# CrazeXD/Prometheus

Hardware: AMD Instinct MI355X
Metric: spectrum points/sec (phase x wavelength) (higher is better)
Workload: dtype f64; 1 GPU; C3 (powerLaw: NaI+CaII+MgI), 351222 wavelengths x 16 phases x 2400 chords x 30 samples; global_wavelengths=351222, orbital_phases=16, chords_per_phase=2400, los_samples=30, parallelism=wavelength shards x1 (no collective)

## Files before the change

### prometheus_amd/csrc/prom_api.hip

```cpp
#include <algorithm>
#include <cstdio>
#include <cstdlib>
#include <cmath>
#include <cstring>
#include <exception>
#include <map>
#include <mutex>
#include <thread>

#include "prom_internal.h"

using prom::DevBuf;
using prom::Error;

namespace {

template <class F>
int32_t guarded(prom_ctx* ctx, F&& f) {
  if (!ctx) return PROM_E_ARG;
  try {
    PROM_HIP(hipSetDevice(ctx->device));
    f();
    ctx->err.clear();
    return PROM_OK;
// ... 699 lines not shown
          double m = 0.0;
          const int64_t cnt = n_orb * tr.n_pr * tr.n_x;
          for (int64_t i = 0; i < cnt; ++i) {
            const double v = std::fabs(S.n_tabulated[i]);
            if (std::isfinite(v) && v > m) m = v;
          }
          nref[sc] = m;
        } else if (S.density.kind == PROM_DENSITY_GRIDDED) {
          int64_t gnx, gny, gnz, glen;
          gridded_dims(S.density, &gnx, &gny, &gnz, &glen);
          double m = 0.0;
          for (int64_t i = gnx + gny + gnz; i < glen; ++i) {
            const double v = std::fabs(S.n_tabulated[i]);
            if (std::isfinite(v) && v > m) m = v;
          }
          nref[sc] = m * (1.0 + 1e-9);
        } else {
          const double* p = S.density.p;
          bool bounded = p[0] >= 0.0 && std::isfinite(p[0]);
          if (S.density.kind == PROM_DENSITY_BAROMETRIC) bounded = bounded && p[2] > 0.0;
          if (S.density.kind == PROM_DENSITY_POWERLAW) bounded = bounded && p[2] >= 0.0 && p[1] > 0.0;
          if (S.density.kind == PROM_DENSITY_HYDROSTATIC)
            bounded = bounded && p[4] >= 0.0 && p[1] > 0.0 && p[3] != 0.0 &&
                      p[4] >= p[2] / (p[3] * p[1]) * (1.0 - 1e-12);
          if (!bounded) tr.window = false;
          nref[sc] = std::fabs(p[0]) * (1.0 + 1e-9);
        }
      }
      for (const auto& t : tr.terms)
        if (!t.is_molecule && !(t.chi >= 0.0)) tr.window = false;
      std::vector<prom::SigTabDev> st;
      for (const auto& t : tr.terms) {
        if (t.is_molecule) continue;
        const prom::AtomTable& tb = ctx->tables[t.table];
        const double bound = std::fabs(t.chi) * nref[t.scenario] * (double)tr.n_x * tr.delta_x;
        const double c = (bound > 0.0 && std::isfinite(bound)) ? 1.0 / bound : 0.0;
        if (!std::isfinite(bound) || (bound > 0.0 && !(c > 0.0))) tr.window = false;
        const double inv = (c > 0.0 && std::isfinite(c)) ? bound : 0.0;
        st.push_back({tb.x.as<double>(), tb.y.as<double>(), tb.n, tb.offset,
                      tr.shift.as<double>() + (int64_t)t.scenario * n_orb, tb.dir.as<int32_t>(), tb.n_dir, 0,
                      tb.dir_x0, tb.dir_inv_h, std::isfinite(c) ? c : 0.0, inv, t.chi, tb.hx.front(), tb.hx.back(),
                      tb.rec.as<double4>()});
      }
      int32_t sc0 = -1;
      bool one_sc = n_atoms >= 2 && n_mol == 0;
      double smax_m = 0.0;
      for (const auto& t : tr.terms) {
        if (t.is_molecule) continue;
        if (sc0 < 0) sc0 = t.scenario;
        if (t.scenario != sc0 || !(std::isfinite(t.chi) && t.chi >= 0.0)) one_sc = false;
        smax_m += t.chi * tr.atom_sigma_max[t.slot];
      }
      tr.species_merge_ok = tr.species_merge_ok && one_sc && tr.n_sc <= 4;
      if (tr.species_merge_ok) {
        const double bound = nref[sc0] * (double)tr.n_x * tr.delta_x;
        const double c = (bound > 0.0 && std::isfinite(bound)) ? 1.0 / bound : 0.0;
        if (!std::isfinite(bound) || (bound > 0.0 && !(c > 0.0)) || !std::isfinite(smax_m)) tr.species_merge_ok = false;
        tr.sigtab_m = prom::SigTabs4{};
        tr.sigtab_m.t[0] = st[0];
        tr.sigtab_m.t[0].ncoef = std::isfinite(c) ? c : 0.0;
        tr.sigtab_m.t[0].nscale = (c > 0.0 && std::isfinite(c)) ? bound : 0.0;
        tr.sigtab_m.t[0].chi = 1.0;
        tr.colargs_m = prom::ColArgs{};
        prom::TermDev tm{};
        tm.scenario = sc0;
        tm.is_molecule = 0;
        tm.slot = 0;
        tm.table = -1;
        tm.chi = 1.0;
        tr.colargs_m.t[0] = tm;
        stg.add(tr.sigma_max_m, &smax_m, 1, s);
        tr.qbound_m = smax_m * tr.sigtab_m.t[0].nscale;
      }
      stg.add(tr.sigtab, st.data(), (int64_t)st.size(), s);
      tr.qbound_v = 0.0;
      for (size_t i = 0; i < st.size(); ++i) tr.qbound_v += tr.atom_sigma_max[i] * st[i].nscale;
      {
        const bool cols8e = n_mol == 0 && tr.n_x <= 64 && (int32_t)tr.terms.size() <= 8 && tr.n_sc <= 4;
        tr.tcurve = tr.tcurve && cols8e && tr.exp_mode && tr.window && !pb->has_star && n_atoms >= 1 &&
                    (n_atoms == 1 || tr.species_merge_ok);
        const double yb = !tr.tcurve ? 0.0 : (n_atoms == 1 ? tr.atom_sigma_max[0] : smax_m);
        const double nb = !tr.tcurve ? 0.0 : (n_atoms == 1 ? st[0].nscale : tr.sigtab_m.t[0].nscale);
        tr.tc_ybound = (std::isfinite(yb) && yb > 0.0) ? yb : 0.0;
        const double qb = yb * nb;
        int lg = prom::kTcMaxOctaves;
        if (std::isfinite(qb) && qb > 0.0) lg = std::max(1, std::min(prom::kTcMaxOctaves, std::ilogb(qb) + 7 + 2));
        if (const char* e = std::getenv("PROM_TC_LG")) lg = std::max(1, std::min(lg, std::atoi(e)));
        tr.tc_lg = lg;
      }
      tr.uniform_shift = !(pb->options & PROM_OPT_DOPPLER_ROWS);
      for (const auto& t : tr.terms) {
        if (t.is_molecule) continue;
        for (int64_t o = 1; o < n_orb; ++o)
          if (!(sh[t.scenario * n_orb + o] == sh[t.scenario * n_orb])) tr.uniform_shift = false;
      }
      tr.sigtab_v = prom::SigTabs4{};
      for (size_t i = 0; i < st.size() && i < 4; ++i) tr.sigtab_v.t[i] = st[i];
      tr.sig_seg_ok = false;
      std::vector<double> key_sh;
      std::vector<uint64_t> key_gen;
      for (const auto& t : tr.terms) {
        if (t.is_molecule) continue;
        key_gen.push_back(ctx->tables[t.table].gen);
        key_sh.insert(key_sh.end(), sh.begin() + t.scenario * n_orb, sh.begin() + (t.scenario + 1) * n_orb);
      }
      const char* srows = std::getenv("PROM_SIGMA_ROWS");
      const bool no_guess = srows && std::atoi(srows) == 0;
      const char* e_sd = std::getenv("PROM_SEG_DIR");
      const bool use_dir = !(e_sd && std::atoi(e_sd) == 0);
      const bool want_seg = true;
      const bool seg_reuse = !no_guess && use_dir && tr.seg_key_valid && key_gen == tr.seg_key_gen &&
                             key_sh == tr.seg_key_sh && (int64_t)tr.seg_key_wav.size() == tr.n_wav &&
                             std::memcmp(tr.seg_key_wav.data(), pb->wavelength, sizeof(double) * tr.n_wav) == 0;
      tr.seg_key_valid = false;
      seg_key_keep = seg_reuse;
      if (!seg_reuse) tr.tw_ok = false;
      const char* e_tw = std::getenv("PROM_TW");
      const bool tw_off = e_tw && std::atoi(e_tw) == 0;
      auto build_tw = [&]() {
        tr.tw_ok = false;
        tr.n_tw = 0;
        std::vector<const std::vector<double>*> tabs;
        int32_t sc_tw = -1;
        bool one = n_orb >= 2;
        for (const auto& t : tr.terms) {
          if (t.is_molecule) continue;
          if (sc_tw < 0) sc_tw = t.scenario;
          for (int64_t o = 0; o < n_orb; ++o)
            if (!(sh[t.scenario * n_orb + o] == sh[sc_tw * n_orb + o])) one = false;
          tabs.push_back(&ctx->tables[t.table].hx);
        }
        if (!one || sc_tw < 0 || tw_off) return;
        static const int rowcap_env = [] { const char* e = std::getenv("PROM_TW_ROWCAP"); return e ? std::max(1, std::atoi(e)) : 0; }();
        const int rowcap = rowcap_env > 0 ? rowcap_env : std::max(256, std::min(768, (int)(4096 / std::max<int64_t>(1, n_orb)) / 64 * 64));
        static const int64_t pmax_env = [] { const char* e = std::getenv("PROM_TW_PMAX"); return e ? (int64_t)std::max(1, std::atoi(e)) : (int64_t)0; }();
        const int64_t pmax = pmax_env > 0 ? pmax_env : std::max<int64_t>(8192, (int64_t)rowcap * n_orb);
        static const int lamcap = [] {
          const char* e = std::getenv("PROM_TW_LAMCAP");
          return e ? std::max(0, std::min(prom::kTwLamCap, std::atoi(e))) : prom::kTwLamCap;
        }();
        static const int lds = [] {
          const char* e = std::getenv("PROM_TW_LDS");
          return e ? std::max(16, std::min(prom::kTwLds, std::atoi(e))) : prom::kTwLds;
        }();
        std::vector<prom::SigSeg> twseg;
        std::vector<int32_t> twrow, twlam;
        int32_t nw = 0;
        if (!prom::build_target_windows(pb->wavelength, tr.n_wav, sh.data() + (int64_t)sc_tw * n_orb, (int32_t)n_orb, tabs,
                                        lds, lamcap, rowcap, pmax, twseg, twrow, twlam, nw))
          return;
        stg.add(tr.tw_seg, twseg.data(), (int64_t)twseg.size(), s);
        stg.add(tr.tw_row, twrow.data(), (int64_t)twrow.size(), s);
        stg.add(tr.tw_lam, twlam.data(), (int64_t)twlam.size(), s);
        tr.n_tw = nw;
        tr.tw_ok = true;
        tr.tw_new = true;
        if (std::getenv("PROM_DEBUG")) {
          int64_t k[4] = {0, 0, 0, 0};
          for (const auto& e : twseg) k[e.kind & 3] += 1;
          int64_t lam_st = 0, lam_n = 0;
          for (int32_t b = 0; b < nw; ++b)
            if (twlam[2 * b + 1] > twlam[2 * b]) {
              ++lam_st;
              lam_n += twlam[2 * b + 1] - twlam[2 * b];
            }
          std::fprintf(stderr, "[prom] target windows: %d (slices: %lld staged, %lld global, %lld staged unguessed, "
                       "%lld outside the table; wavelengths staged in %lld windows, %.1f per window)\n", nw,
                       (long long)k[1], (long long)k[2], (long long)k[3], (long long)k[0], (long long)lam_st,
                       lam_st ? (double)lam_n / (double)lam_st : 0.0);
        }
      };
      if (seg_reuse) {
        tr.sig_seg_ok = true;
        if (tw_off) tr.tw_ok = false;
        else if (!tr.tw_ok) build_tw();
      } else if (want_seg && n_atoms >= 1 && n_atoms <= 4) {
        tr.seg_key_valid = false;
        const int64_t nb = (tr.n_wav + prom::kSigBlockW - 1) / prom::kSigBlockW;
        std::vector<prom::SigSeg> seg(nb * n_atoms, prom::SigSeg{0, 0, 0, 0, 0.0, 0.0});
        std::vector<prom::SigSeg> seg4(nb * n_atoms * 4, prom::SigSeg{0, 0, 0, 0, 0.0, 0.0});
        std::vector<prom::SigSeg> segr;
        std::vector<int32_t> sdir;
        std::mutex segr_mu;
        int32_t ia = 0;
        for (const auto& t : tr.terms) {
          if (t.is_molecule) continue;
          const prom::AtomTable& tb = ctx->tables[t.table];
          const std::vector<double>& X = tb.hx;
          const int64_t n = tb.n;
          double smin = INFINITY, smax = -INFINITY;
          bool ok = n >= 2 && (int64_t)X.size() == n;
          for (int64_t o = 0; o < n_orb; ++o) {
            const double v = sh[t.scenario * n_orb + o];
            if (!(v > 0.0) || !std::isfinite(v)) ok = false;
            smin = std::min(smin, v);
            smax = std::max(smax, v);
          }
          auto bracket = [&](double v) -> int64_t {
            int64_t j = (int64_t)(std::upper_bound(X.begin(), X.end(), v) - X.begin()) - 1;
            return j < 0 ? 0 : (j > n - 2 ? n - 2 : j);
          };
          auto make_seg = [&](double tlo, double thi, prom::SigSeg& e) -> bool {
            const int64_t lo = bracket(tlo);
            const int64_t hi = bracket(thi) + 1;
            const int64_t m = hi - lo + 1;
            if (m < 2 || m > INT32_MAX / 2) return false;
            e.lo = (int32_t)lo;
            e.m = (int32_t)m;
            const double xs = X[lo], span = X[hi] - X[lo];
            const double inv = span > 0.0 ? (double)(m - 1) / span : 0.0;
            const double b0 = -(xs * inv);
            bool lin = span > 0.0 && std::isfinite(inv) && std::isfinite(b0);
            auto guess = [&](double v) -> int64_t {
              const double f = std::fma(v, inv, b0);
              int64_t g = f < 0.0 ? 0 : (f >= (double)(m - 2) ? m - 2 : (int64_t)f);
              return g;
            };
            for (int64_t i = lo; lin && i < hi; ++i) {
              if (X[i] == X[i + 1]) continue;
              const double a = std::max(X[i], tlo), z = std::nextafter(X[i + 1], -INFINITY);
              if (a > z) continue;
              const int64_t k = i - lo;
              const int64_t ga = guess(a), gz = guess(z);
              if (ga < k - 1 || ga > k + 1 || gz < k - 1 || gz > k + 1) lin = false;
            }
            e.kind = 0;
            if (lin) {
              e.kind = (m <= prom::kSigSeg ? 1 : 2) | (m <= prom::tc_slice_cap(n_atoms) ? 64 : 0);
              e.xs = b0;
              e.inv = inv;
            }
            return true;
          };
          auto blocks = [&](int64_t b0, int64_t b1) {
          for (int64_t b = b0; ok && b < b1; ++b) {
            double lmin = INFINITY, lmax = -INFINITY;
            bool fin = true;
            for (int64_t w = b * prom::kSigBlockW; w < std::min<int64_t>(tr.n_wav, (b + 1) * prom::kSigBlockW); ++w) {
              const double l = pb->wavelength[w];
              if (!(l > 0.0) || !std::isfinite(l)) fin = false;
              lmin = std::min(lmin, l);
              lmax = std::max(lmax, l);
            }
            if (!fin) continue;
            const double tlo = smin * lmin, thi = smax * lmax;
            if (!(tlo >= X[0] && thi < X[n - 1])) continue;
            prom::SigSeg& e = seg[b * n_atoms + ia];
            if (!make_seg(tlo, thi, e)) continue;
            if ((e.kind & 3) == 0) {
              bool any = false;
              for (int q = 0; q < prom::kSigBlockW / 64; ++q) {
                double wl = INFINITY, wh = -INFINITY;
                const int64_t w0 = b * prom::kSigBlockW + 64 * q;
                for (int64_t w = w0; w < std::min<int64_t>(tr.n_wav, w0 + 64); ++w) {
                  wl = std::min(wl, pb->wavelength[w]);
                  wh = std::max(wh, pb->wavelength[w]);
                }
                prom::SigSeg& ew = seg4[(b * n_atoms + ia) * 4 + q];
                if (wl <= wh && make_seg(smin * wl, smax * wh, ew) && (ew.kind & 3) != 0) {
                  ew.kind = 2;
                  any = true;
                } else {
                  ew = prom::SigSeg{0, 0, 0, 0, 0.0, 0.0};
                }
              }
              if (any) e.kind |= 8;
              if (!use_dir) continue;
              const int64_t lo = e.lo, m = e.m, hi = lo + m - 1;
              const double x0 = X[lo], span = X[hi] - X[lo];
              if (!(span > 0.0)) continue;
              std::vector<int32_t> dv;
              prom::SigSeg de{(int32_t)lo, 0, 32, 0, 0.0, 0.0};
              bool okd = false;
              for (int64_t mult = 4; !okd && mult <= 1024 && m * mult <= (1 << 22); mult *= 4) {
                const int64_t B = m * mult;
                const double inv = (double)B / span, b0 = -(x0 * inv);
                if (!std::isfinite(inv) || !std::isfinite(b0)) break;
                dv.assign(B, 0);
                int64_t k = 0;
                for (int64_t j = 0; j < B; ++j) {
                  const double v = x0 + span * ((double)j / (double)B);
                  while (k < m - 2 && X[lo + k + 1] <= v) ++k;
                  dv[j] = (int32_t)k;
                }
                auto gd = [&](double v) -> int64_t {
                  const double f = std::fma(v, inv, b0);
                  const int64_t j = f < 0.0 ? 0 : (f >= (double)(B - 1) ? B - 1 : (int64_t)f);
                  return dv[j];
                };
                okd = true;
                for (int64_t o = 0; okd && o < n_orb; ++o) {
                  const double v = sh[t.scenario * n_orb + o];
                  for (int64_t w = b * prom::kSigBlockW; okd && w < (b + 1) * prom::kSigBlockW; ++w) {
                    const double tt = v * pb->wavelength[std::min<int64_t>(w, tr.n_wav - 1)];
                    const int64_t kk = bracket(tt) - lo, g = gd(tt);
                    if (kk < 0 || kk > m - 2 || g < kk - 1 || g > kk + 1) okd = false;
                  }
                }
                if (okd) {
                  de.m = (int32_t)(B + 1);
                  de.xs = b0;
                  de.inv = inv;
                }
              }
              if (okd) {
                std::lock_guard<std::mutex> lk(segr_mu);
// ... 626 lines not shown
```

### prometheus_amd/csrc/prom_internal.h

```cpp
#pragma once

#include <hip/hip_runtime.h>

#include <cstdint>
#include <stdexcept>
#include <string>
#include <vector>

#include "../../include/prom_hip.h"

namespace prom {

struct Error : std::runtime_error {
  int32_t code;
  Error(int32_t c, const std::string& m) : std::runtime_error(m), code(c) {}
};

#define PROM_HIP(expr)                                                                      \
  do {                                                                                      \
    hipError_t _e = (expr);                                                                 \
    if (_e != hipSuccess)                                                                   \
      throw ::prom::Error(PROM_E_HIP, std::string(#expr) + ": " + hipGetErrorString(_e));   \
  } while (0)

// ... 141 lines not shown

struct SigTabs4 {
  SigTabDev t[4];
};

constexpr int kTcHdr = 16;
constexpr int kTcD = 16;
enum : int { kTcHNmax = 0, kTcHTfrac = 1, kTcHFsum = 2, kTcHT0 = 3 ,
             kTcHL = 9, kTcHFlags = 10 , kTcHNact = 11 };
constexpr int kTcMaxOctaves = 64;
constexpr int kTcChain = 4;
constexpr int kTcPartMax = 16;
constexpr int kTcPartVals = (kTcChain + 1) * kTcD;

struct TcArgs {
  const double* hdr;
  const double* tab;
  const int32_t* flags;
  const double* ncol;
  const double* fout;
  double* R;
  unsigned long long* evals;
  int32_t lg, n_pr;
};

struct AtomTable {
  bool live = false;
  DevBuf x, y;
  int64_t n = 0;
  double offset = 0.0;
  double ymax = 0.0;
  DevBuf dir;
  DevBuf rec;
  double amax = 0.0;
  std::vector<double> hx;
  int32_t n_dir = 0;
  double dir_x0 = 0.0, dir_inv_h = 0.0;
  uint64_t gen = 0;
};

struct MolTable {
  bool live = false;
  DevBuf P, T, W, V;
  int32_t n_p = 0, n_t = 0;
  int64_t n_w = 0;
  double offset = 0.0;
  double vmax = 0.0;
};

constexpr int kMaxSlots = 8;
struct RunSlot {
  DevBuf ncol;
  DevBuf flags;
  DevBuf recs;
  DevBuf act_ip;
  DevBuf counts;
  DevBuf tsum;
  DevBuf fsum;
  DevBuf mrecs;
  DevBuf wenv;
  DevBuf wmom;
  DevBuf evals;
  DevBuf sig;
  DevBuf ntot;
  DevBuf molcol;
  DevBuf mol_smp;
  DevBuf mol_nin;
  DevBuf mol_lst;
  DevBuf mol_rend;
  DevBuf zfl;
  DevBuf tq;
  DevBuf trec;
  DevBuf hlist;
  DevBuf hcnt;
  DevBuf R;
  DevBuf tc_hdr;
  DevBuf tc_tab;
  DevBuf tc_part;
  DevBuf tc_cnt;
  DevBuf tc_pp;
  hipStream_t aux = nullptr;
  hipEvent_t ev_fork = nullptr, ev_join = nullptr;
  bool sig_late = false;
};

struct TransitDev {
  int64_t n_wav = 0;
  int32_t n_pr = 0, n_orb = 0, n_x = 0, n_sc = 0, n_moons = 0;
  int32_t n_atoms = 0, n_mol = 0, n_terms = 0;
  double delta_x = 0.0, planet_R = 0.0, cull_tau = 0.0;
  bool ready = false;
  bool ran = false;
  std::vector<TermDev> terms;
  std::vector<DensityDev> dens;
  std::vector<double> atom_sigma_max;
  std::vector<double> mol_T;
  DevBuf wav, cy, cz, cfout, x, planet_y, moon_y, moon_R;
  DevBuf body_x, body_y, shift;
  DevBuf dens_dev;
  DevBuf scdev;
  DevBuf terms_dev;
  DevBuf tab;
  DevBuf sigma;
  DevBuf sigma_max_dev;
  DevBuf sigtab;
  SigTabs4 sigtab_v{};
  ColArgs colargs{};
  int32_t exp_mode = 1;
  bool merge = true;
  bool window = true;
  bool uniform_shift = false;
  bool count_evals = false;
  bool plan = true;
  bool species_merge_ok = false;
  ColArgs colargs_m{};
  SigTabs4 sigtab_m{};
  DevBuf sigma_max_m;
  double qbound_v = 0.0, qbound_m = 0.0;
  int32_t taup_resident = 0;
  unsigned long long* ts_out = nullptr;
  int32_t ts_cap = 0;
  int32_t ts_blocks = 0;
  hipEvent_t* kprof = nullptr;
  uint32_t kprof_mask = 0;
  DevBuf molslot;
  DevBuf mirror;
  int64_t n_mirror = 0;
  bool mol_stage = true;
  std::vector<int32_t> mirror_h;
  DevBuf sig_seg4;
  int64_t sig_noguess = 0;
  DevBuf sig_dir;
  DevBuf rm_fout;
  DevBuf rm_ftab;
  bool rm_ftab_ok = false;
  DevBuf mol_g;
  std::vector<MolSlotDev> mslots;
  std::vector<int64_t> tab_off;
  int32_t star_table_id = -1;
  bool star = false;
  bool star_uniform = false;
  SigTabDev star_tab{};
  DevBuf crho, cclv, cshift;
  DevBuf rm_slices;
  DevBuf sig_seg;
  DevBuf sig_fb;
  int32_t n_sig_fb = 0;
  DevBuf sig_fb_tc;
  int32_t n_sig_fb_tc = 0;
  bool sig_seg_ok = false;
  DevBuf tw_seg;
  DevBuf tw_row;
  DevBuf tw_lam;
  int32_t n_tw = 0;
  bool tw_ok = false;
  bool tw_new = false;
  int32_t sig_deg = 0;
  DevBuf sig_flags;
  std::vector<double> seg_key_wav, seg_key_sh;
  std::vector<uint64_t> seg_key_gen;
  bool seg_key_valid = false;
  bool tcurve = true;
  int32_t tc_lg = 1;
  DevBuf tc_const;
  int32_t tc_parts = 1;
  double tc_fsum = 0.0;
  bool tc_pp_ok = false;
  double tc_ybound = 0.0;
  RunSlot slot[kMaxSlots];
  hipGraphExec_t gexec[kMaxSlots] = {};
  bool graphs = false;
  int8_t env_fork = -1;
  bool env_stagger = false;
  int depth = 1;
  int cu_count = 0;
  int last = 0;
};

}

struct prom_ctx {
  int32_t device = 0;
  hipStream_t stream = nullptr;
  hipStream_t streams[prom::kMaxSlots] = {};
  int pipeline = 4;
  hipEvent_t ev[8] = {};
  std::string err;
  std::vector<prom::AtomTable> tables;
  std::vector<prom::MolTable> mtables;
  prom::TransitDev tr;
  prom::DevBuf scratch[6];
  bool timing = false;
  std::vector<hipEvent_t> tev;
  std::vector<prom::DevBuf> tsbuf;
  std::vector<int32_t> ts_blocks;
  int32_t timed_runs = 0;
  int32_t timing_stride = 1;
  int64_t window_runs = 0;
  void* pin = nullptr;
  size_t pin_cap = 0;
  std::vector<hipEvent_t> pin_ev;
  hipEvent_t fork_ev[prom::kMaxSlots] = {}, join_ev[prom::kMaxSlots] = {};
  uint64_t table_gen = 0;
  void* upin = nullptr;
  size_t upin_cap = 0;
  prom::DevBuf ustage;
};

namespace prom {

void launch_table_lookup(hipStream_t s, const double* x, const double* y, int64_t n, double offset,
                         const double* targets, int64_t nt, double* out);
void launch_voigt(hipStream_t s, const double* x, int64_t n, const double* lw, const double* lg,
                  const double* lc, int32_t nl, double sigma_v, double c_light, double offset,
                  int log_table, double* out);
void launch_density(hipStream_t s, const DensityDev& m, const double* x, int32_t n_x, const double* y,
                    const double* z, const double* bx, const double* by, int64_t n_chords, double* out);
void launch_molecular_sigma(hipStream_t s, const MolTable& t, int64_t n_chords, int32_t n_x,
                            const double* P, double T, int64_t n_wav, const double* wav, double* out);
void launch_transit(hipStream_t s, TransitDev& tr, RunSlot& rs, const std::vector<AtomTable>& tables,
                    const std::vector<MolTable>& mtables, hipEvent_t* ev, int* variant, bool stage_events);
void launch_sigma_rows(hipStream_t s, int32_t nsig, const SigTabs4& tabv, const double* wav, int64_t n_wav,
                       int32_t n_rows, const SigSeg* seg, const int32_t* fb, int32_t n_fb, double* sig, float4* tq,
                       int32_t merge_sp, double nscale_m, uint8_t* zfl, hipEvent_t ev_start, hipEvent_t ev_stop);
void launch_sigma_poly(hipStream_t s, int32_t nsig, int32_t deg, const SigTabs4& tabv, const double* wav, int64_t n_wav,
                       int32_t n_rows, const SigSeg* seg, const int32_t* fb, int32_t n_fb, double* sig, float4* tq,
                       int32_t merge_sp, double nscale_m, uint8_t* zfl, hipEvent_t ev_start, hipEvent_t ev_stop);
void launch_seg_exact(hipStream_t s, int32_t nsig, const SigTabs4& tabv, const double* wav, int64_t n_wav,
                      int32_t n_rows, SigSeg* seg, int32_t* flags);
bool launch_tcurve(hipStream_t s, TransitDev& tr, RunSlot& rs, int32_t nsig, bool msp, hipEvent_t ev_sig0,
                   hipEvent_t ev_sig1, hipEvent_t ev_tb0, hipEvent_t ev_tb1);
void launch_tau_mol(hipStream_t s, TransitDev& tr, RunSlot& rs, int32_t na, dim3 g, int32_t ppg);
void launch_mol_gt(hipStream_t s, const MolSlotDev& md);
void launch_rm_fout(hipStream_t s, TransitDev& tr);
void launch_tau_rm(hipStream_t s, TransitDev& tr, RunSlot& rs, int32_t na, hipEvent_t* ev);
double reduce_max(hipStream_t s, const double* v, int64_t n, double* scratch_dev);
void launch_gridded(hipStream_t s, const double* g, int32_t nx, int32_t ny, int32_t nz, int64_t n,
                    const double* px, const double* py, const double* pz, double* out);
void launch_sigma_tw(hipStream_t s, TransitDev& tr, int32_t nsig, int32_t deg, const TcArgs& ta, hipEvent_t ev0,
                     hipEvent_t ev1);
void launch_tw_exact(hipStream_t s, TransitDev& tr, int32_t nsig);
bool build_target_windows(const double* wav, int64_t n_wav, const double* shift, int32_t n_rows,
                          const std::vector<const std::vector<double>*>& tabs, int32_t lds, int32_t lamcap,
                          int32_t rowcap, int64_t pmax, std::vector<SigSeg>& seg_out, std::vector<int32_t>& row_out,
                          std::vector<int32_t>& lam_out, int32_t& n_win);
void launch_table_recs(hipStream_t s, const double* x, const double* y, int64_t n, double4* rec, double* amax);
void launch_scatter(hipStream_t s, const char* base, const ScatterDesc* d, int32_t n);
void launch_band_stats(hipStream_t s, const double* R, const double* wav, int32_t n_orb, int64_t n_wav,
                       int32_t n_bands, const double* bounds, double* sum, int64_t* count, double* mx);
void launch_star_disk(hipStream_t s, const SigTabDev& tb, const double* shift, const double* clv, const double* rho,
                      int32_t n_cells, double dphi, double drho, const double* wav, int64_t n_wav, double* out);

}
```

### prometheus_amd/csrc/prom_tc.h

```cpp
#pragma once
#include "prom_device.h"

namespace prom {

constexpr double kTcEps = 0x1p-7;
constexpr int kTcExpEps = -7;
constexpr double kTcSat = 40.0;

__device__ __forceinline__ int32_t tc_exponent(double q) {
  return (int32_t)((__builtin_bit_cast(unsigned long long, q) >> 52) & 0x7ff) - 1023;
}

__device__ __forceinline__ int32_t tc_octaves(double qhi) {
  if (!(qhi >= kTcEps)) return 0;
  if (!(qhi <= 1.0e300)) return 0x7fffffff;
  return tc_exponent(qhi) - kTcExpEps + 1;
}

__device__ __forceinline__ double tc_clenshaw(double q, const double* __restrict__ c) {
  const double m = __builtin_bit_cast(double, (__builtin_bit_cast(unsigned long long, q) & 0x000fffffffffffffull) |
                                                  0x3ff0000000000000ull);
  const double u = __builtin_fma(2.0, log2(m), -1.0);
  double b1 = 0.0, b2 = 0.0, c0 = 0.0;
#pragma unroll 1
  for (int k0 = kTcD - 4; k0 >= 0; k0 -= 4) {
    const double2 ca = *reinterpret_cast<const double2*>(c + k0), cb = *reinterpret_cast<const double2*>(c + k0 + 2);
    const double cv[4] = {ca.x, ca.y, cb.x, cb.y};
#pragma unroll
    for (int i = 3; i >= 0; --i) {
      if (k0 + i >= 1) {
        const double b0 = __builtin_fma(2.0 * u, b1, cv[i] - b2);
        b2 = b1;
        b1 = b0;
      } else {
        c0 = cv[0];
      }
    }
  }
  return __builtin_fma(u, b1, c0 - b2);
}

#ifndef PROM_TC_CS_ATTR
#define PROM_TC_CS_ATTR __noinline__ __attribute__((optnone))
#endif
__device__ PROM_TC_CS_ATTR double tc_chord_sum(double Y, bool nf, bool zr, double fs,
                                                                    const int32_t* __restrict__ fl,
                                                                    const double* __restrict__ nc,
                                                                    const double* __restrict__ fout, int32_t n_pr) {
  const double inv_fs = 1.0 / fs;
  double a = 0.0;
  for (int32_t ci = 0; ci < n_pr; ++ci) {
    if (fl[ci] != 0) continue;
    const double N = nc[ci];
    double tau = N * Y;
    if (nf && zr && !__builtin_isfinite(N)) tau = __builtin_nan("");
    const double e = exp(-tau);
    a = nf ? a + fout[ci] * e : a + (fout[ci] * inv_fs) * e;
  }
  return a;
}

__device__ __forceinline__ double tc_eval(double Y, const double* __restrict__ h, const double* __restrict__ tabo,
                                          const int32_t* __restrict__ fl, const double* __restrict__ nc,
                                          const double* __restrict__ fout, int32_t n_pr, unsigned long long* evals) {
  const double q = Y * h[kTcHNmax];
  const double tf = h[kTcHTfrac];
  if (q < kTcEps) {
    double p = h[kTcHT0 + 5];
#pragma unroll
    for (int e = 4; e >= 0; --e) p = __builtin_fma(p, q, h[kTcHT0 + e]);
    return tf + p;
  }
  const int32_t nact = (int32_t)h[kTcHNact];
  if (!(q == q)) return nact > 0 ? q : tf;
  const int32_t L = (int32_t)h[kTcHL];
  const int32_t j = q <= 1.0e300 ? tc_exponent(q) - kTcExpEps : 0x7fffffff;
  if (j < L) return tf + tc_clenshaw(q, tabo + (int64_t)j * kTcD);
  if ((int32_t)h[kTcHFlags] & 1) return tf;
  const double inv_fs = 1.0 / h[kTcHFsum];
  double a = 0.0;
#pragma unroll 1
  for (int32_t c = 0; c < n_pr; ++c)
    if (fl[c] == 0) a += (fout[c] * inv_fs) * exp(-(nc[c] * Y));
  if (evals) atomicAdd(&evals[threadIdx.x & 63], (unsigned long long)nact);
  return tf + a;
}

__device__ __forceinline__ double fma_s(double a, double b, double c) {
  double r;
  asm("v_fma_f64 %0, %1, %2, %3" : "=v"(r) : "v"(a), "v"(b), "s"(c));
  return r;
}

__device__ __forceinline__ double tc_eval_full_s(double Y, const double* __restrict__ h, const double* __restrict__ tabo) {
  const double q = Y * h[kTcHNmax];
  const double tf = h[kTcHTfrac];
  if (q < kTcEps) {
    double c5 = h[kTcHT0 + 5];
    asm volatile("" : "+v"(c5));
    double p = fma_s(c5, q, h[kTcHT0 + 4]);
#pragma unroll
    for (int e = 3; e >= 0; --e) p = fma_s(p, q, h[kTcHT0 + e]);
    return tf + p;
  }
  const int32_t nact = (int32_t)h[kTcHNact];
  if (!(q == q)) return nact > 0 ? q : tf;
  const int32_t L = (int32_t)h[kTcHL];
  const int32_t j = q <= 1.0e300 ? tc_exponent(q) - kTcExpEps : 0x7fffffff;
  if (j >= L) return tf;
  return tf + tc_clenshaw(q, tabo + (int64_t)j * kTcD);
}

__device__ __forceinline__ double tc_eval_full(double Y, const double* __restrict__ h, const double* __restrict__ tabo) {
  const double q = Y * h[kTcHNmax];
  const double tf = h[kTcHTfrac];
  if (q < kTcEps) {
    double p = h[kTcHT0 + 5];
#pragma unroll
    for (int e = 4; e >= 0; --e) p = __builtin_fma(p, q, h[kTcHT0 + e]);
    return tf + p;
  }
  const int32_t nact = (int32_t)h[kTcHNact];
  if (!(q == q)) return nact > 0 ? q : tf;
  const int32_t L = (int32_t)h[kTcHL];
  const int32_t j = q <= 1.0e300 ? tc_exponent(q) - kTcExpEps : 0x7fffffff;
  if (j >= L) return tf;
  return tf + tc_clenshaw(q, tabo + (int64_t)j * kTcD);
}

}
```

### prometheus_amd/csrc/prom_tw.hip

```cpp
#include "prom_tc.h"

namespace prom {


template <int NSIG, int D, bool MG, int RP>
__global__ void __launch_bounds__(kBlock) k_sigma_tw(const SigTabs4 tabv, const SigTabDev* __restrict__ tabp,
                                                     const PolyCoef pc, const double* __restrict__ wav,
                                                     int64_t n_wav, int32_t n_rows, const SigSeg* __restrict__ wseg,
                                                     const int32_t* __restrict__ wrow, const int32_t* __restrict__ wlam,
                                                     int32_t n_win, const TcArgs ta,
                                                     const double* __restrict__ hdr, const double* __restrict__ shift,
                                                     const double* __restrict__ ctab, double* __restrict__ Rout) {
  static_assert(D > 0, "polynomial lookups only (coarse tables take k_sigma_tc)");
  __shared__ double2 lds2[kTwLds / 2 + 32];
  double* const lds = reinterpret_cast<double*>(lds2);
  const int32_t per = (n_win + 7) >> 3;
  const int32_t b = (int32_t)(blockIdx.x & 7) * per + (int32_t)(blockIdx.x >> 3);
  if (b >= n_win) return;
  const int tid = threadIdx.x, lane = tid & 63;
  const int32_t wv = __builtin_amdgcn_readfirstlane(tid >> 6);
  SigSeg sg[NSIG];
  bool wrare = false;
  bool wexact = true;
  bool wsearch = false;
  int32_t tot = 0;
#pragma unroll
  for (int s = 0; s < NSIG; ++s) {
    sg[s] = wseg[(int64_t)b * NSIG + s];
    wrare = wrare || ((sg[s].kind & 3) != 1 && (sg[s].kind & 3) != 3);
    wsearch = wsearch || (sg[s].kind & 3) == 3;
    wexact = wexact && (sg[s].kind & 4) != 0;
    if (sg[s].kind & 1) tot = sg[s].pad + sg[s].m > tot ? sg[s].pad + sg[s].m : tot;
  }
  const int32_t lw0 = wlam[2 * b], nlam = wlam[2 * b + 1] - lw0;
  double2* const sel = lds2;
  double* const sx = lds + 2 * tot;
  double* const slam = sx + tot + NSIG;
  {
    constexpr int NQ = (kTwLds / 3 + kBlock - 1) / kBlock;
    constexpr int NL = (kTwLamCap + kBlock - 1) / kBlock;
    double lq[NL];
#pragma unroll
    for (int j = 0; j < NL; ++j) {
      const int32_t i = tid + j * kBlock;
      lq[j] = i < nlam ? wav[lw0 + i] : 0.0;
    }
    double4 q[NQ];
    int sp[NQ];
#pragma unroll
    for (int j = 0; j < NQ; ++j) {
      const int32_t i = tid + j * kBlock;
      sp[j] = -1;
#pragma unroll
      for (int s = 0; s < NSIG; ++s)
        if ((sg[s].kind & 1) && i >= sg[s].pad && i < sg[s].pad + sg[s].m) sp[j] = s;
      int32_t gi = 0;
      const double4* __restrict__ rr = tabv.t[0].rec;
#pragma unroll
      for (int s = 0; s < NSIG; ++s)
        if (sp[j] == s) {
          gi = sg[s].lo + (i - sg[s].pad);
          rr = tabv.t[s].rec;
        }
      q[j] = i < tot ? rr[gi] : make_double4(0.0, 0.0, 0.0, 0.0);
    }
#pragma unroll
    for (int j = 0; j < NQ; ++j) {
      const int32_t i = tid + j * kBlock;
#pragma unroll
      for (int s = 0; s < NSIG; ++s) {
        if (sp[j] != s) continue;
        sx[i + s] = q[j].x;
        sel[i] = make_double2(MG ? tabv.t[s].chi * q[j].y : q[j].y, q[j].z);
        if (i == sg[s].pad + sg[s].m - 1) sx[i + s + 1] = q[j].w;
      }
    }
#pragma unroll
    for (int j = 0; j < NL; ++j) {
      const int32_t i = tid + j * kBlock;
      if (i < nlam) slam[i] = lq[j];
    }
  }
  __syncthreads();
  double choff = 0.0;
  if constexpr (MG) {
#pragma unroll
    for (int s = 0; s < NSIG; ++s) choff += tabv.t[s].chi * tabv.t[s].offset;
  }
  const int32_t* __restrict__ wa = wrow + (int64_t)b * n_rows;
  const int32_t* __restrict__ wz = wa + n_rows;
  if (!wrare) {
    const double* xsb[NSIG];
    const double2* elb[NSIG];
    double xsv[NSIG];
#pragma unroll
    for (int s = 0; s < NSIG; ++s) {
      xsb[s] = sx + sg[s].pad + s;
      elb[s] = sel + sg[s].pad;
      xsv[s] = sg[s].xs;
      asm volatile("" : "+v"(xsv[s]));
    }
    double cdv = pc.c[D];
    asm volatile("" : "+v"(cdv));
    const double* lamb = slam + lane - lw0;
    struct RowS {
      const double* h;
      const double* tabo;
      double* Rrow;
      double sh;
      int32_t w0, w1;
    };
    auto row_of = [&](int32_t o) {
      RowS r;
      r.h = hdr + (int64_t)o * kTcHdr;
      r.tabo = ctab + (int64_t)o * ta.lg * kTcD;
      r.Rrow = Rout + (int64_t)o * n_wav + lane;
      r.sh = shift[o];
      r.w0 = wa[o];
      r.w1 = wz[o];
      return r;
    };
    auto chunk = [&](const RowS* rs, auto np_tag, const int32_t* c0, const double* lam, auto mode_tag) {
      constexpr int NP = decltype(np_tag)::value;
      constexpr int MODE = decltype(mode_tag)::value;
      constexpr bool EX = MODE == 0;
      double t[NP];
#pragma unroll
      for (int p = 0; p < NP; ++p) t[p] = rs[p].sh * lam[p];
      int32_t g[NP][NSIG];
      double x0[NP][NSIG], x1[NP][NSIG];
      double2 e[NP][NSIG];
#pragma unroll
      for (int p = 0; p < NP; ++p)
#pragma unroll
        for (int s = 0; s < NSIG; ++s) {
          g[p][s] = min((int32_t)__builtin_fma(t[p], sg[s].inv, xsv[s]), sg[s].m - 2);
          x0[p][s] = xsb[s][g[p][s]];
          if constexpr (!EX) x1[p][s] = xsb[s][g[p][s] + 1];
          e[p][s] = elb[s][g[p][s]];
        }
      if constexpr (!EX) {
#pragma unroll
        for (int p = 0; p < NP; ++p)
#pragma unroll
          for (int s = 0; s < NSIG; ++s) {
            if (MODE == 2 && (sg[s].kind & 3) == 3) {
              int32_t k = 0;
              for (int32_t st = 1 << (31 - __builtin_clz((uint32_t)(sg[s].m - 1) | 1u)); st > 0; st >>= 1)
                if (k + st <= sg[s].m - 2 && xsb[s][k + st] <= t[p]) k += st;
              x0[p][s] = xsb[s][k];
              e[p][s] = elb[s][k];
              continue;
            }
            const bool lo = t[p] < x0[p][s], hi = t[p] >= x1[p][s];
            if (lo | hi) {
              const int32_t k = lo ? g[p][s] - 1 : g[p][s] + 1;
              x0[p][s] = xsb[s][k];
              e[p][s] = elb[s][k];
            }
          }
      }
      double acc[NP];
#pragma unroll
      for (int p = 0; p < NP; ++p) {
        acc[p] = 0.0;
#pragma unroll
        for (int s = 0; s < NSIG; ++s) {
          const double a = e[p][s].y * (t[p] - x0[p][s]);
          double q = __builtin_fma(cdv, a, pc.c[D - 1]);
#pragma unroll
          for (int k = D - 2; k >= 0; --k) q = __builtin_fma(q, a, pc.c[k]);
          if constexpr (MG) acc[p] = __builtin_fma(e[p][s].x, q, acc[p]);
          else acc[p] = __builtin_fma(e[p][s].x, q, -tabv.t[s].offset);
        }
        if constexpr (MG) acc[p] -= choff;
      }
#pragma unroll
      for (int p = 0; p < NP; ++p) {
        const double v = tc_eval_full_s(acc[p], rs[p].h, rs[p].tabo);
        if (c0[p] + lane < rs[p].w1) rs[p].Rrow[c0[p]] = v;
      }
    };
    auto rows = [&](const RowS* rs, auto np_tag, int32_t k0, int32_t G, auto mode_tag) {
      constexpr int NP = decltype(np_tag)::value;
      int32_t nch = 0;
#pragma unroll
      for (int p = 0; p < NP; ++p) nch = max(nch, (rs[p].w1 - rs[p].w0 + 63) >> 6);
      auto cfix = [&](int p, int32_t c) { return c < rs[p].w1 ? c : rs[p].w0; };
      if (nlam > 0) {
        for (int32_t k = k0; k < nch; k += G) {
          int32_t c0[NP];
          double lam[NP];
#pragma unroll
          for (int p = 0; p < NP; ++p) {
            c0[p] = rs[p].w0 + 64 * k;
            lam[p] = lamb[cfix(p, c0[p])];
          }
          chunk(rs, np_tag, c0, lam, mode_tag);
        }
      } else {
        constexpr int B = 4 / NP;
        for (int32_t k = k0; k < nch; k += B * G) {
          double lam[B][NP];
#pragma unroll
          for (int j = 0; j < B; ++j)
#pragma unroll
            for (int p = 0; p < NP; ++p) {
              const int32_t w = cfix(p, rs[p].w0 + 64 * (k + j * G)) + lane;
              lam[j][p] = wav[w < rs[p].w1 ? w : rs[p].w1 - 1];
            }
#pragma unroll
          for (int j = 0; j < B; ++j) {
            if (k + j * G >= nch) break;
            int32_t c0[NP];
#pragma unroll
            for (int p = 0; p < NP; ++p) c0[p] = rs[p].w0 + 64 * (k + j * G);
            chunk(rs, np_tag, c0, lam[j], mode_tag);
          }
        }
      }
    };
    auto rows_mode = [&](const RowS* rs, auto np_tag, int32_t k0, int32_t G) {
      if (wexact) rows(rs, np_tag, k0, G, std::integral_constant<int, 0>{});
      else if (!wsearch) rows(rs, np_tag, k0, G, std::integral_constant<int, 1>{});
      else rows(rs, np_tag, k0, G, std::integral_constant<int, 2>{});
    };
    auto rare_row = [&](int32_t o) { return ((int32_t)hdr[(int64_t)o * kTcHdr + kTcHFlags] & 6) != 0; };
    if constexpr (RP == 1) {
      const int32_t G = n_rows >= 4 ? 1 : (n_rows == 1 ? 4 : 2);
      for (int32_t o = __builtin_amdgcn_readfirstlane(wv / G); o < n_rows; o += 4 / G) {
        if (rare_row(o)) continue;
        const RowS r1[1] = {row_of(o)};
        rows_mode(r1, std::integral_constant<int, 1>{}, wv % G, G);
      }
    } else {
      const int32_t P = (n_rows + 1) >> 1;
      const int32_t G = P >= 4 ? 1 : (P == 1 ? 4 : 2);
      for (int32_t q = __builtin_amdgcn_readfirstlane(wv / G); q < P; q += 4 / G) {
        const int32_t oa = 2 * q, ob = 2 * q + 1;
        const bool ra = rare_row(oa), rb = ob >= n_rows || rare_row(ob);
        if (!ra && !rb) {
          const RowS r2[2] = {row_of(oa), row_of(ob)};
          rows_mode(r2, std::integral_constant<int, 2>{}, wv % G, G);
        } else if (!ra || !rb) {
          const RowS r1[1] = {row_of(ra ? ob : oa)};
          rows_mode(r1, std::integral_constant<int, 1>{}, wv % G, G);
        }
      }
    }
  }
  auto run_pass = [&](auto pass_tag) {
    constexpr int pass = decltype(pass_tag)::value;
    auto next_item = [&](int32_t& o, int32_t& c, int32_t& w0, int32_t& w1) {
      o = __builtin_amdgcn_readfirstlane(o);
      c = __builtin_amdgcn_readfirstlane(c);
      while (o < n_rows) {
        const bool rare = wrare || ((int32_t)hdr[(int64_t)o * kTcHdr + kTcHFlags] & 6) != 0;
        if (rare == (pass == 1)) {
          w0 = __builtin_amdgcn_readfirstlane(wa[o]);
          w1 = __builtin_amdgcn_readfirstlane(wz[o]);
          const int32_t nch = (w1 - w0 + 63) >> 6;
          if (c < nch) return;
          c = __builtin_amdgcn_readfirstlane(c - nch);
        }
        o = __builtin_amdgcn_readfirstlane(o + 1);
      }
    };
    int32_t on = 0, cn = wv, w0n = 0, w1n = 0;
    next_item(on, cn, w0n, w1n);
    while (on < n_rows) {
      const int32_t o = __builtin_amdgcn_readfirstlane(on), w1 = __builtin_amdgcn_readfirstlane(w1n);
      const int32_t w = __builtin_amdgcn_readfirstlane(w0n + cn * 64) + lane;
      const bool live = w < w1;
      const double lam = wav[live ? w : w1 - 1];
      cn += 4;
      next_item(on, cn, w0n, w1n);
      const double t = shift[o] * lam;
      const double* h = hdr + (int64_t)o * kTcHdr;
      double acc = 0.0, v;
      {
        bool zr = false;
#pragma unroll
        for (int s = 0; s < NSIG; ++s) {
          const SigTabDev& tb = tabp[s];
          if (t >= tb.xfirst && t < tb.xlast) {
            const double4 q = tb.rec[bracket_of(t, tb)];
            const double ex = exp_taylor<D>(q.z * (t - q.x), pc);
            if constexpr (MG) {
              acc = __builtin_fma(tb.chi * q.y, ex, acc);
              zr = zr || !(tb.chi * __builtin_fma(q.y, ex, -tb.offset) > 0.0);
            } else {
              acc = __builtin_fma(q.y, ex, -tb.offset);
            }
          } else {
            const double sv = sigma_poly_of(t, tb, pc, D);
            if constexpr (MG) {
              acc = __builtin_fma(tb.chi, sv + tb.offset, acc);
              zr = zr || !(tb.chi * sv > 0.0);
            } else {
              acc = sv;
            }
          }
        }
        if constexpr (MG) acc -= choff;
        const double Y = acc;
        const bool nf = ((int32_t)h[kTcHFlags] & 2) != 0;
        const double q = Y * h[kTcHNmax];
        const int32_t L = (int32_t)h[kTcHL];
        const int32_t j = q <= 1.0e300 ? tc_exponent(q) - kTcExpEps : 0x7fffffff;
        const bool beyond = !nf && q >= kTcEps && q == q && j >= L && !((int32_t)h[kTcHFlags] & 1);
        if (!nf && !beyond) {
          v = tc_eval_full(Y, h, ctab + (int64_t)o * ta.lg * kTcD);
        } else {
          const double fs = h[kTcHFsum];
          const double a = tc_chord_sum(Y, nf, zr, fs, ta.flags + (int64_t)o * ta.n_pr, ta.ncol + (int64_t)o * ta.n_pr,
                                        ta.fout, ta.n_pr);
          if (beyond && ta.evals) atomicAdd(&ta.evals[threadIdx.x & 63], (unsigned long long)(int32_t)h[kTcHNact]);
          v = nf ? (a + h[kTcHTfrac] * fs) / fs : h[kTcHTfrac] + a;
        }
      }
      if (live) Rout[(int64_t)o * n_wav + w] = v;
    }
  };
  run_pass(std::integral_constant<int, 1>{});
}

template <int NSIG>
__global__ void __launch_bounds__(kBlock) k_tw_exact(const SigTabs4 tabv, const double* __restrict__ wav,
                                                     int32_t n_rows, SigSeg* __restrict__ wseg,
                                                     const int32_t* __restrict__ wrow) {
  const int32_t b = blockIdx.x;
  const int32_t* wa = wrow + (int64_t)b * n_rows;
  const int32_t* wz = wa + n_rows;
  __shared__ int32_t bad;
  if (threadIdx.x == 0) bad = 0;
  __syncthreads();
  bool ok = true;
  for (int32_t o = 0; o < n_rows; ++o) {
    const int32_t w0 = wa[o], w1 = wz[o];
    for (int32_t w = w0 + (int32_t)threadIdx.x; w < w1; w += kBlock) {
      const double t = tabv.t[0].shift[o] * wav[w];
#pragma unroll
      for (int s = 0; s < NSIG; ++s) {
        const SigSeg sg = wseg[(int64_t)b * NSIG + s];
        if ((sg.kind & 3) != 1) continue;
        const int32_t g = seg_guess(t, sg.xs, sg.inv, sg.m);
        const double* __restrict__ X = tabv.t[s].x + sg.lo;
        int32_t a = 0, c = sg.m - 1;
        while (c - a > 1) {
          const int32_t mid = (a + c) >> 1;
          if (X[mid] <= t) a = mid; else c = mid;
        }
        ok = ok && a == g;
      }
    }
  }
  if (!ok) bad = 1;
  __syncthreads();
  if (threadIdx.x < NSIG && !bad) {
    SigSeg& sg = wseg[(int64_t)b * NSIG + threadIdx.x];
    if ((sg.kind & 3) == 1) sg.kind |= 4;
  }
}

void launch_tw_exact(hipStream_t s, TransitDev& tr, int32_t nsig) {
  if (!tr.tw_ok || tr.n_tw <= 0) return;
  SigSeg* twseg = tr.tw_seg.as<SigSeg>();
  const int32_t* twrow = tr.tw_row.as<int32_t>();
#define PROM_TWE(NS)                                                                                            \
  hipLaunchKernelGGL((k_tw_exact<NS>), dim3((unsigned)tr.n_tw), dim3(kBlock), 0, s, tr.sigtab_v, tr.wav.as<double>(), \
                     tr.n_orb, twseg, twrow)
  switch (nsig) {
    case 1: PROM_TWE(1); break;
    case 2: PROM_TWE(2); break;
    case 3: PROM_TWE(3); break;
    default: PROM_TWE(4); break;
  }
#undef PROM_TWE
  PROM_HIP(hipGetLastError());
}

void launch_sigma_tw(hipStream_t s, TransitDev& tr, int32_t nsig, int32_t deg, const TcArgs& ta, hipEvent_t ev0,
                     hipEvent_t ev1) {
  const unsigned nbw = (unsigned)(((int64_t)tr.n_tw + 7) / 8 * 8);
  const SigSeg* twseg = tr.tw_seg.as<SigSeg>();
  const int32_t* twrow = tr.tw_row.as<int32_t>();
  const int32_t* twlam = tr.tw_lam.as<int32_t>();
  const PolyCoef& pc = poly_coef();
  const SigTabs4& tabv = tr.sigtab_v;
  const SigTabDev* tabp = tr.sigtab.as<SigTabDev>();
  const double* wav = tr.wav.as<double>();
  const int32_t n_rows = tr.n_orb;
  const int64_t n_wav = tr.n_wav;
  PROM_REQUIRE(deg > 0 && n_rows >= 2 && tr.n_tw > 0, "k_sigma_tw: polynomial lookups with orbital Doppler rows");
  static const int rp_env = [] { const char* e = std::getenv("PROM_TW_RP"); return e ? std::atoi(e) : 0; }();
  const int rp = rp_env == 1 || rp_env == 2 ? rp_env : (nsig == 1 ? 2 : 1);
#define PROM_TWK(NS, DG, MGV)                                                                                        \
  if (rp == 2)                                                                                                       \
    hipExtLaunchKernelGGL((k_sigma_tw<NS, DG, MGV, 2>), dim3(nbw), dim3(kBlock), 0, s, ev0, ev1, 0, tabv, tabp, pc, wav, \
                          n_wav, n_rows, twseg, twrow, twlam, tr.n_tw, ta, ta.hdr, tabv.t[0].shift, ta.tab, ta.R);   \
  else                                                                                                               \
    hipExtLaunchKernelGGL((k_sigma_tw<NS, DG, MGV, 1>), dim3(nbw), dim3(kBlock), 0, s, ev0, ev1, 0, tabv, tabp, pc, wav, \
                          n_wav, n_rows, twseg, twrow, twlam, tr.n_tw, ta, ta.hdr, tabv.t[0].shift, ta.tab, ta.R)
#define PROM_TWD(NS, MGV)                 \
  if (deg <= 8) { PROM_TWK(NS, 8, MGV); } \
  else { PROM_TWK(NS, 14, MGV); }
  switch (nsig) {
    case 1: PROM_TWD(1, false) break;
    case 2: PROM_TWD(2, true) break;
    case 3: PROM_TWD(3, true) break;
    default: PROM_TWD(4, true) break;
  }
#undef PROM_TWD
#undef PROM_TWK
  PROM_HIP(hipGetLastError());
}

}
```

Baseline: 173.7 billion spectrum points/s.

## Schedule target windows by cost and add wave-uniform Clenshaw evaluation

The host estimates a per-window cost, sorts windows largest-first within each of eight stripes, and passes a permutation to k_sigma_tw. The permutation is used only when the window count exceeds the number of resident blocks, so heavy blocks start first and the tail is shorter. Several kernel tweaks ride along: Chebyshev table evaluation serialised per unique table index across the wave, so coefficient loads become scalar and uniform; prefetch of the next wavelength; a v_med3 clamp; an explicit waitcnt; and skipping empty rows in paired mode. The costs are an extra indirection, a host-side sort, and a ballot loop that can serialise when lanes hit many different octaves.

```diff
diff --git a/prometheus_amd/csrc/prom_api.hip b/prometheus_amd/csrc/prom_api.hip
--- a/prometheus_amd/csrc/prom_api.hip
+++ b/prometheus_amd/csrc/prom_api.hip
@@ -875,6 +875,28 @@
         stg.add(tr.tw_seg, twseg.data(), (int64_t)twseg.size(), s);
         stg.add(tr.tw_row, twrow.data(), (int64_t)twrow.size(), s);
         stg.add(tr.tw_lam, twlam.data(), (int64_t)twlam.size(), s);
+        static const int order_env = [] { const char* e = std::getenv("PROM_TW_ORDER"); return e ? std::atoi(e) : 1; }();
+        std::vector<int32_t> twperm((size_t)nw);
+        {
+          const int32_t na = (int32_t)tabs.size();
+          std::vector<int64_t> cost((size_t)nw);
+          for (int32_t b = 0; b < nw; ++b) {
+            int64_t c = twlam[2 * b + 1] - twlam[2 * b];
+            for (int64_t o = 0; o < n_orb; ++o)
+              c += 64 * (((int64_t)twrow[(int64_t)(b + 1) * n_orb + o] - twrow[(int64_t)b * n_orb + o] + 63) / 64);
+            for (int32_t a = 0; a < na; ++a)
+              if (twseg[(int64_t)b * na + a].kind & 1) c += twseg[(int64_t)b * na + a].m;
+            cost[b] = c;
+            twperm[b] = b;
+          }
+          const int32_t per = (nw + 7) >> 3;
+          for (int32_t x0 = 0; order_env != 0 && x0 < nw; x0 += per) {
+            const auto a = twperm.begin() + x0, z = twperm.begin() + std::min(nw, x0 + per);
+            std::stable_sort(a, z, [&](int32_t i, int32_t j) { return cost[i] > cost[j]; });
+            if (order_env < 0) std::reverse(a, z);
+          }
+        }
+        stg.add(tr.tw_perm, twperm.data(), (int64_t)twperm.size(), s);
         tr.n_tw = nw;
         tr.tw_ok = true;
         tr.tw_new = true;
diff --git a/prometheus_amd/csrc/prom_internal.h b/prometheus_amd/csrc/prom_internal.h
--- a/prometheus_amd/csrc/prom_internal.h
+++ b/prometheus_amd/csrc/prom_internal.h
@@ -317,6 +317,7 @@
   DevBuf tw_seg;
   DevBuf tw_row;
   DevBuf tw_lam;
+  DevBuf tw_perm;
   int32_t n_tw = 0;
   bool tw_ok = false;
   bool tw_new = false;
diff --git a/prometheus_amd/csrc/prom_tc.h b/prometheus_amd/csrc/prom_tc.h
--- a/prometheus_amd/csrc/prom_tc.h
+++ b/prometheus_amd/csrc/prom_tc.h
@@ -111,6 +111,60 @@
   return tf + tc_clenshaw(q, tabo + (int64_t)j * kTcD);
 }
 
+__device__ __forceinline__ double tc_clenshaw_wave(bool on, int32_t j, double u, double fall, double r,
+                                                   const double* __restrict__ tabo) {
+  unsigned long long todo = __ballot(on);
+  while (todo != 0) {
+    const int32_t ju = __builtin_amdgcn_readlane(j, (int32_t)__builtin_ctzll(todo));
+    const double* __restrict__ c = tabo + (int64_t)ju * kTcD;
+    double b1 = 0.0, b2 = 0.0, c0 = 0.0;
+#pragma unroll 1
+    for (int k0 = kTcD - 4; k0 >= 0; k0 -= 4) {
+      const double cv[4] = {c[k0], c[k0 + 1], c[k0 + 2], c[k0 + 3]};
+#pragma unroll
+      for (int i = 3; i >= 0; --i) {
+        if (k0 + i >= 1) {
+          const double b0 = __builtin_fma(2.0 * u, b1, cv[i] - b2);
+          b2 = b1;
+          b1 = b0;
+        } else {
+          c0 = cv[0];
+        }
+      }
+    }
+    const bool mine = on && j == ju;
+    if (mine) r = fall + __builtin_fma(u, b1, c0 - b2);
+    todo &= ~__ballot(mine);
+  }
+  return r;
+}
+
+__device__ __forceinline__ double tc_eval_full_w(double Y, bool live, const double* __restrict__ h,
+                                                 const double* __restrict__ tabo) {
+  const double q = Y * h[kTcHNmax];
+  const double tf = h[kTcHTfrac];
+  const int32_t L = (int32_t)h[kTcHL];
+  const int32_t j = q <= 1.0e300 ? tc_exponent(q) - kTcExpEps : 0x7fffffff;
+  const bool tail = q < kTcEps;
+  const bool on = live && !tail && q == q && j < L;
+  double r = tf, u = 0.0;
+  if (tail) {
+    double c5 = h[kTcHT0 + 5];
+    asm volatile("" : "+v"(c5));
+    double p = fma_s(c5, q, h[kTcHT0 + 4]);
+#pragma unroll
+    for (int e = 3; e >= 0; --e) p = fma_s(p, q, h[kTcHT0 + e]);
+    r = tf + p;
+  } else if (!(q == q)) {
+    r = (int32_t)h[kTcHNact] > 0 ? q : tf;
+  } else if (on) {
+    const double m = __builtin_bit_cast(double, (__builtin_bit_cast(unsigned long long, q) & 0x000fffffffffffffull) |
+                                                    0x3ff0000000000000ull);
+    u = __builtin_fma(2.0, log2(m), -1.0);
+  }
+  return tc_clenshaw_wave(on, j, u, tf, r, tabo);
+}
+
 __device__ __forceinline__ double tc_eval_full(double Y, const double* __restrict__ h, const double* __restrict__ tabo) {
   const double q = Y * h[kTcHNmax];
   const double tf = h[kTcHTfrac];
diff --git a/prometheus_amd/csrc/prom_tw.hip b/prometheus_amd/csrc/prom_tw.hip
--- a/prometheus_amd/csrc/prom_tw.hip
+++ b/prometheus_amd/csrc/prom_tw.hip
@@ -2,21 +2,28 @@
 
 namespace prom {
 
+
+__device__ __forceinline__ int32_t med3_s(int32_t g, int32_t hi) {
+  int32_t r;
+  asm("v_med3_i32 %0, %1, 0, %2" : "=v"(r) : "v"(g), "s"(hi));
+  return r;
+}
 
 template <int NSIG, int D, bool MG, int RP>
 __global__ void __launch_bounds__(kBlock) k_sigma_tw(const SigTabs4 tabv, const SigTabDev* __restrict__ tabp,
                                                      const PolyCoef pc, const double* __restrict__ wav,
                                                      int64_t n_wav, int32_t n_rows, const SigSeg* __restrict__ wseg,
                                                      const int32_t* __restrict__ wrow, const int32_t* __restrict__ wlam,
-                                                     int32_t n_win, const TcArgs ta,
+                                                     const int32_t* __restrict__ wperm, int32_t n_win, const TcArgs ta,
                                                      const double* __restrict__ hdr, const double* __restrict__ shift,
                                                      const double* __restrict__ ctab, double* __restrict__ Rout) {
   static_assert(D > 0, "polynomial lookups only (coarse tables take k_sigma_tc)");
   __shared__ double2 lds2[kTwLds / 2 + 32];
   double* const lds = reinterpret_cast<double*>(lds2);
   const int32_t per = (n_win + 7) >> 3;
-  const int32_t b = (int32_t)(blockIdx.x & 7) * per + (int32_t)(blockIdx.x >> 3);
-  if (b >= n_win) return;
+  const int32_t slot = (int32_t)(blockIdx.x & 7) * per + (int32_t)(blockIdx.x >> 3);
+  if (slot >= n_win) return;
+  const int32_t b = wperm ? wperm[slot] : slot;
   const int tid = threadIdx.x, lane = tid & 63;
   const int32_t wv = __builtin_amdgcn_readfirstlane(tid >> 6);
   SigSeg sg[NSIG];
@@ -134,7 +141,7 @@
       for (int p = 0; p < NP; ++p)
 #pragma unroll
         for (int s = 0; s < NSIG; ++s) {
-          g[p][s] = min((int32_t)__builtin_fma(t[p], sg[s].inv, xsv[s]), sg[s].m - 2);
+          g[p][s] = med3_s((int32_t)__builtin_fma(t[p], sg[s].inv, xsv[s]), sg[s].m - 2);
           x0[p][s] = xsb[s][g[p][s]];
           if constexpr (!EX) x1[p][s] = xsb[s][g[p][s] + 1];
           e[p][s] = elb[s][g[p][s]];
@@ -177,8 +184,9 @@
       }
 #pragma unroll
       for (int p = 0; p < NP; ++p) {
-        const double v = tc_eval_full_s(acc[p], rs[p].h, rs[p].tabo);
-        if (c0[p] + lane < rs[p].w1) rs[p].Rrow[c0[p]] = v;
+        const bool live = c0[p] + lane < rs[p].w1;
+        const double v = tc_eval_full_w(acc[p], live, rs[p].h, rs[p].tabo);
+        if (live) rs[p].Rrow[c0[p]] = v;
       }
     };
     auto rows = [&](const RowS* rs, auto np_tag, int32_t k0, int32_t G, auto mode_tag) {
@@ -187,14 +195,19 @@
 #pragma unroll
       for (int p = 0; p < NP; ++p) nch = max(nch, (rs[p].w1 - rs[p].w0 + 63) >> 6);
       auto cfix = [&](int p, int32_t c) { return c < rs[p].w1 ? c : rs[p].w0; };
+      if (k0 >= nch) return;
       if (nlam > 0) {
+        double lamn[NP];
+#pragma unroll
+        for (int p = 0; p < NP; ++p) lamn[p] = lamb[cfix(p, rs[p].w0 + 64 * k0)];
         for (int32_t k = k0; k < nch; k += G) {
           int32_t c0[NP];
           double lam[NP];
 #pragma unroll
           for (int p = 0; p < NP; ++p) {
             c0[p] = rs[p].w0 + 64 * k;
-            lam[p] = lamb[cfix(p, c0[p])];
+            lam[p] = lamn[p];
+            lamn[p] = lamb[cfix(p, c0[p] + 64 * G)];
           }
           chunk(rs, np_tag, c0, lam, mode_tag);
         }
@@ -209,6 +222,7 @@
               const int32_t w = cfix(p, rs[p].w0 + 64 * (k + j * G)) + lane;
               lam[j][p] = wav[w < rs[p].w1 ? w : rs[p].w1 - 1];
             }
+          __builtin_amdgcn_s_waitcnt(0x0f70);
 #pragma unroll
           for (int j = 0; j < B; ++j) {
             if (k + j * G >= nch) break;
@@ -226,6 +240,7 @@
       else rows(rs, np_tag, k0, G, std::integral_constant<int, 2>{});
     };
     auto rare_row = [&](int32_t o) { return ((int32_t)hdr[(int64_t)o * kTcHdr + kTcHFlags] & 6) != 0; };
+    auto empty_row = [&](int32_t o) { return wa[o] >= wz[o]; };
     if constexpr (RP == 1) {
       const int32_t G = n_rows >= 4 ? 1 : (n_rows == 1 ? 4 : 2);
       for (int32_t o = __builtin_amdgcn_readfirstlane(wv / G); o < n_rows; o += 4 / G) {
@@ -238,7 +253,7 @@
       const int32_t G = P >= 4 ? 1 : (P == 1 ? 4 : 2);
       for (int32_t q = __builtin_amdgcn_readfirstlane(wv / G); q < P; q += 4 / G) {
         const int32_t oa = 2 * q, ob = 2 * q + 1;
-        const bool ra = rare_row(oa), rb = ob >= n_rows || rare_row(ob);
+        const bool ra = rare_row(oa) || empty_row(oa), rb = ob >= n_rows || rare_row(ob) || empty_row(ob);
         if (!ra && !rb) {
           const RowS r2[2] = {row_of(oa), row_of(ob)};
           rows_mode(r2, std::integral_constant<int, 2>{}, wv % G, G);
@@ -380,6 +395,18 @@
   PROM_HIP(hipGetLastError());
 }
 
+template <int NSIG, int D, bool MG, int RP>
+static int32_t tw_resident() {
+  static const int32_t n = [] {
+    int dev = 0, cus = 0, per_cu = 0;
+    PROM_HIP(hipGetDevice(&dev));
+    PROM_HIP(hipDeviceGetAttribute(&cus, hipDeviceAttributeMultiprocessorCount, dev));
+    PROM_HIP(hipOccupancyMaxActiveBlocksPerMultiprocessor(&per_cu, k_sigma_tw<NSIG, D, MG, RP>, kBlock, 0));
+    return (int32_t)(cus * per_cu);
+  }();
+  return n;
+}
+
 void launch_sigma_tw(hipStream_t s, TransitDev& tr, int32_t nsig, int32_t deg, const TcArgs& ta, hipEvent_t ev0,
                      hipEvent_t ev1) {
   const unsigned nbw = (unsigned)(((int64_t)tr.n_tw + 7) / 8 * 8);
@@ -395,13 +422,16 @@
   PROM_REQUIRE(deg > 0 && n_rows >= 2 && tr.n_tw > 0, "k_sigma_tw: polynomial lookups with orbital Doppler rows");
   static const int rp_env = [] { const char* e = std::getenv("PROM_TW_RP"); return e ? std::atoi(e) : 0; }();
   const int rp = rp_env == 1 || rp_env == 2 ? rp_env : (nsig == 1 ? 2 : 1);
+  const int32_t* twperm = nullptr;
 #define PROM_TWK(NS, DG, MGV)                                                                                        \
+  twperm = tr.n_tw > (rp == 2 ? tw_resident<NS, DG, MGV, 2>() : tw_resident<NS, DG, MGV, 1>())                       \
+               ? tr.tw_perm.as<int32_t>() : nullptr;                                                                 \
   if (rp == 2)                                                                                                       \
     hipExtLaunchKernelGGL((k_sigma_tw<NS, DG, MGV, 2>), dim3(nbw), dim3(kBlock), 0, s, ev0, ev1, 0, tabv, tabp, pc, wav, \
-                          n_wav, n_rows, twseg, twrow, twlam, tr.n_tw, ta, ta.hdr, tabv.t[0].shift, ta.tab, ta.R);   \
+                          n_wav, n_rows, twseg, twrow, twlam, twperm, tr.n_tw, ta, ta.hdr, tabv.t[0].shift, ta.tab, ta.R);   \
   else                                                                                                               \
     hipExtLaunchKernelGGL((k_sigma_tw<NS, DG, MGV, 1>), dim3(nbw), dim3(kBlock), 0, s, ev0, ev1, 0, tabv, tabp, pc, wav, \
-                          n_wav, n_rows, twseg, twrow, twlam, tr.n_tw, ta, ta.hdr, tabv.t[0].shift, ta.tab, ta.R)
+                          n_wav, n_rows, twseg, twrow, twlam, twperm, tr.n_tw, ta, ta.hdr, tabv.t[0].shift, ta.tab, ta.R)
 #define PROM_TWD(NS, MGV)                 \
   if (deg <= 8) { PROM_TWK(NS, 8, MGV); } \
   else { PROM_TWK(NS, 14, MGV); }
```

After: 165.8 billion spectrum points/s. -4.5%, worse.
